# pxl-th/SLAM.jl

Hardware: AMD Instinct MI355X
Metric: frames/sec KITTI-05 stereo @1k kpts; local-BA ms/iter for 50-KF window (higher is better)
Workload: dtype f64

## Files before the change

slam.jl_amd/csrc/pyramid.hip:

```cpp
#include "common.hpp"
#include <cmath>
#include <cstdlib>
#include <mutex>
#include <tuple>
#include <utility>

#define LINE_THREADS 64

struct PlaneSet {
    double *p[4];
    const double *nrm[4];
    int coef[4];
    int fill0[4];
    const double *sq[4];
    int n;
    size_t zs;
};
#define PS_PICK(ps, f, pl) ((pl) == 0 ? (ps).f[0] : (pl) == 1 ? (ps).f[1] : (pl) == 2 ? (ps).f[2] : (ps).f[3])
__device__ __forceinline__ double *ps_plane(const PlaneSet &ps, int pl) { return PS_PICK(ps, p, pl) + (size_t)blockIdx.z * ps.zs; }
__device__ __forceinline__ const double *ps_nrm(const PlaneSet &ps, int pl) { return PS_PICK(ps, nrm, pl); }
__device__ __forceinline__ int ps_coef(const PlaneSet &ps, int pl) { return PS_PICK(ps, coef, pl); }
__device__ __forceinline__ bool ps_fill0(const PlaneSet &ps, int pl) { return PS_PICK(ps, fill0, pl) != 0; }
__device__ __forceinline__ const double *ps_sq(const PlaneSet &ps, int pl) { const double *q = PS_PICK(ps, sq, pl); return q ? q + (size_t)blockIdx.z * ps.zs : nullptr; }

// ... 236 lines not shown
    });
    const double uplus = iplus / k.inv1masum;
    const double vplus = uplus / k.inv1mbsum;
    const double d0 = w1 - uplus, d1 = w2 - uplus, d2 = w3 - uplus;
    const double vr0 = ((k.M[0] * d0 + k.M[1] * d1) + k.M[2] * d2) + vplus;
    const double vr1 = ((k.M[3] * d0 + k.M[4] * d1) + k.M[5] * d2) + vplus;
    const double vr2 = ((k.M[6] * d0 + k.M[7] * d1) + k.M[8] * d2) + vplus;
    double vA = vr0;
    double vB = ((w2 + a1 * vA) + a2 * vr1) + a3 * vr2;
    double vC = ((w3 + a1 * vB) + a2 * vA) + a3 * vr1;
    double v1 = vC, v2 = vB, v3 = vA;
    const double scale = k.scale;
    io.fence();
    if (nrm) {
        io.st(n - 1, (vA * scale) / nrm[(long)(n - 1) * nrm_s]);
        io.st(n - 2, (vB * scale) / nrm[(long)(n - 2) * nrm_s]);
        io.st(n - 3, (vC * scale) / nrm[(long)(n - 3) * nrm_s]);
        for (int i = n - 4; i >= 0; i--) {
            const double t = ((io.ld_dst(i) + a1 * v1) + a2 * v2) + a3 * v3;
            io.st(i, (t * scale) / nrm[(long)i * nrm_s]);
            v3 = v2; v2 = v1; v1 = t;
        }
        return;
    }
    io.st(n - 1, vA * scale); io.st(n - 2, vB * scale); io.st(n - 3, vC * scale);
    io.template sweep<-1>(n - 4, n - 3, true, [&](double x) {
        const double t = ((x + a1 * v1) + a2 * v2) + a3 * v3;
        v3 = v2; v2 = v1; v1 = t;
        return t * scale;
    });
}

template <int NB>
__global__ __launch_bounds__(LINE_THREADS) void k_iir_cols(PlaneSet ps, const double *src0, int H, int W, int P, IIRPair cf)
{
    if (src0) src0 += (size_t)blockIdx.z * ps.zs;
    __shared__ __attribute__((aligned(16))) double tile[64 * COL_LS];
    const int pl = blockIdx.y;
    ColIO<NB> io;
    io.dst = ps_plane(ps, pl); io.src = (pl == 0 && src0) ? src0 : io.dst;
    io.H = H; io.W = W; io.P = P; io.x0 = blockIdx.x * LINE_THREADS; io.lds = tile; io.slo = 0; io.shi = W - 1;
    iir_line(io, H, ps_coef(ps, pl) == 0 ? cf.c[0] : cf.c[1], ps_fill0(ps, pl), nullptr, 0);
}

__global__ __launch_bounds__(LINE_THREADS) void k_iir_rows(PlaneSet ps, int H, int W, int P, IIRPair cf)
{
    const int y = blockIdx.x * LINE_THREADS + threadIdx.x, pl = blockIdx.y;
    if (y >= H) return;
    RowIO io; io.src = ps_plane(ps, pl) + y; io.dst = ps_plane(ps, pl) + y; io.s = P;
    const double *nrm = ps_nrm(ps, pl);
    iir_line(io, W, ps_coef(ps, pl) == 0 ? cf.c[0] : cf.c[1], ps_fill0(ps, pl), nrm ? nrm + y : nullptr, P);
}

#define CK_B 32
struct RowResize { double *dst; int Hd, Wd, Pd; };
__device__ __forceinline__ double dpp_pair_next(double v)
{
    int lo = __double2loint(v), hi = __double2hiint(v);
    lo = __builtin_amdgcn_update_dpp(0, lo, 0xF5, 0xF, 0xF, true);
    hi = __builtin_amdgcn_update_dpp(0, hi, 0xF5, 0xF, 0xF, true);
    return __hiloint2double(hi, lo);
}
#define RCK_LD(ptr) __builtin_nontemporal_load(ptr)
#define RCK_ST(ptr, v) __builtin_nontemporal_store(v, ptr)
#define CK_LD(ptr) (*(ptr))
#define CK_ST(ptr, v) (*(ptr) = (v))
__global__ __launch_bounds__(LINE_THREADS) void k_iir_rows_ck(PlaneSet ps, int H, int W, int P, IIRPair cf, double *ck, RowResize rz)
{
    const int y = blockIdx.x * LINE_THREADS + threadIdx.x, pl = blockIdx.y;
    if (y >= H) return;
    const bool resize = pl == 0 && rz.dst != nullptr;
    const double rsx = (double)W / (double)(rz.Wd > 0 ? rz.Wd : 1), rox = 1 - 0.5 - rsx * (1 - 0.5);
    int xo = rz.Wd, c0 = -1; double fx = 0.0, tprev = 0.0;
    double *rzp = resize ? rz.dst + (size_t)blockIdx.z * ps.zs + (y >> 1) : nullptr;
    const bool exact2 = 2 * rz.Wd == W;
    auto rz_target = [&]() {
        if (xo < 1) { c0 = -1; return; }
        if (exact2) { c0 = 2 * xo - 2; fx = 0.5; return; }
        const double c = rsx * xo + rox;
        int ixx = (int)floor(c);
        if (ixx > W - 1) ixx = W - 1;
        if (ixx < 1) ixx = 1;
        fx = c - ixx;
        c0 = __builtin_amdgcn_readfirstlane(ixx - 1);
    };
    if (resize) rz_target();
    auto emit = [&](int x, double val) {
        if (x == c0) {
            const double h = (1 - fx) * val + fx * tprev;
            const double hn = dpp_pair_next(h);
            const double fy = 0.5;
            const double o = (1 - fy) * h + fy * hn;
            if ((y & 1) == 0) rzp[(size_t)(xo - 1) * rz.Pd] = o;
            xo--; rz_target();
        }
        tprev = val;
    };
    const size_t nlines = (size_t)gridDim.z * gridDim.y * gridDim.x * LINE_THREADS;
    const size_t lineid = ((size_t)blockIdx.z * gridDim.y + pl) * gridDim.x * LINE_THREADS + y;
    double *p = ps_plane(ps, pl) + y;
    const long s = P;
    const int n = W;
    const IIRCoef &k = ps_coef(ps, pl) == 0 ? cf.c[0] : cf.c[1];
    const bool fill0 = ps_fill0(ps, pl);
    const double a1 = k.a1, a2 = k.a2, a3 = k.a3, scale = k.scale;
    const double x0 = p[0];
    const double iminus = fill0 ? 0.0 : x0, iplus = fill0 ? 0.0 : p[(long)(n - 1) * s];
    const double uminus = iminus / k.inv1masum;
    const double o0 = ((x0 + a1 * uminus) + a2 * uminus) + a3 * uminus;
    const double o1 = ((p[s] + a1 * o0) + a2 * uminus) + a3 * uminus;
    const double o2 = ((p[2 * s] + a1 * o1) + a2 * o0) + a3 * uminus;
    const int m = n - 6, nb = (m + CK_B - 1) / CK_B;
    double w3 = o0, w2 = o1, w1 = o2;
    double cur[CK_B], nxt[CK_B];
    auto load_x = [&](int j, double *buf) {
        const double *q = p + (long)(3 + j * CK_B) * s;
        const int len = n - (3 + j * CK_B);
        if (len >= CK_B) {
#pragma unroll
            for (int e = 0; e < CK_B; e++) buf[e] = RCK_LD(q + (long)e * s);
        } else {
#pragma unroll
            for (int e = 0; e < CK_B; e++) buf[e] = e < len ? q[(long)e * s] : 0.0;
        }
    };
    const int nfull = (n - 3) / CK_B;
    const int rem = (n - 3) - nfull * CK_B;
    load_x(0, cur);
    for (int j = 0; j < nfull; j++) {
        load_x(j + 1, nxt);
        if (j > 0 && j < nb) { double *c = ck + ((size_t)j * 3) * nlines + lineid; CK_ST(c, w1); CK_ST(c + nlines, w2); CK_ST(c + 2 * nlines, w3); }
#pragma unroll
        for (int e = 0; e < CK_B; e++) { const double t = ((cur[e] + a1 * w1) + a2 * w2) + a3 * w3; w3 = w2; w2 = w1; w1 = t; }
#pragma unroll
        for (int e = 0; e < CK_B; e++) cur[e] = nxt[e];
    }
    {
        if (nfull > 0 && nfull < nb) { double *c = ck + ((size_t)nfull * 3) * nlines + lineid; CK_ST(c, w1); CK_ST(c + nlines, w2); CK_ST(c + 2 * nlines, w3); }
#pragma unroll
        for (int e = 0; e < CK_B; e++)
            if (e < rem) { const double t = ((cur[e] + a1 * w1) + a2 * w2) + a3 * w3; w3 = w2; w2 = w1; w1 = t; }
    }
    const bool have_last = nfull == nb - 1;
    const double uplus = iplus / k.inv1masum, vplus = uplus / k.inv1mbsum;
    const double d0 = w1 - uplus, d1 = w2 - uplus, d2 = w3 - uplus;
    const double vr0 = ((k.M[0] * d0 + k.M[1] * d1) + k.M[2] * d2) + vplus;
    const double vr1 = ((k.M[3] * d0 + k.M[4] * d1) + k.M[5] * d2) + vplus;
    const double vr2 = ((k.M[6] * d0 + k.M[7] * d1) + k.M[8] * d2) + vplus;
    const double vA = vr0;
    const double vB = ((w2 + a1 * vA) + a2 * vr1) + a3 * vr2;
    const double vC = ((w3 + a1 * vB) + a2 * vA) + a3 * vr1;
    double v1 = vC, v2 = vB, v3 = vA;
    __builtin_amdgcn_fence(__ATOMIC_RELEASE, "workgroup"); __builtin_amdgcn_fence(__ATOMIC_ACQUIRE, "workgroup");
    if (resize) { emit(n - 1, vA * scale); emit(n - 2, vB * scale); emit(n - 3, vC * scale); }
    else { p[(long)(n - 1) * s] = vA * scale; p[(long)(n - 2) * s] = vB * scale; p[(long)(n - 3) * s] = vC * scale; }
    double f1n = 0, f2n = 0, f3n = 0, f1 = 0, f2 = 0, f3 = 0;
    auto load_ck = [&](int j, double &g1, double &g2, double &g3) {
        if (j > 0) { const double *c = ck + ((size_t)j * 3) * nlines + lineid; g1 = CK_LD(c); g2 = CK_LD(c + nlines); g3 = CK_LD(c + 2 * nlines); }
        else { g1 = o2; g2 = o1; g3 = o0; }
    };
    if (nb > 0) {
        const int j = nb - 1, a = 3 + j * CK_B, len = m - j * CK_B;
        if (!have_last) load_x(j, cur);
        load_ck(j, f1, f2, f3);
        if (j > 0) { load_x(j - 1, nxt); load_ck(j - 1, f1n, f2n, f3n); }
#pragma unroll
        for (int e = 0; e < CK_B; e++)
            if (e < len) { const double t = ((cur[e] + a1 * f1) + a2 * f2) + a3 * f3; f3 = f2; f2 = f1; f1 = t; cur[e] = t; }
#pragma unroll
        for (int e = CK_B - 1; e >= 0; e--)
            if (e < len) { const double t = ((cur[e] + a1 * v1) + a2 * v2) + a3 * v3; v3 = v2; v2 = v1; v1 = t; cur[e] = t * scale; if (resize) emit(a + e, cur[e]); }
        double *q = p + (long)a * s;
        if (!resize) {
#pragma unroll
            for (int e = 0; e < CK_B; e++) if (e < len) RCK_ST(q + (long)e * s, cur[e]);
        }
#pragma unroll
        for (int e = 0; e < CK_B; e++) cur[e] = nxt[e];
        f1 = f1n; f2 = f2n; f3 = f3n;
    }
    for (int j = nb - 2; j >= 0; j--) {
        if (j > 0) { load_x(j - 1, nxt); load_ck(j - 1, f1n, f2n, f3n); }
#pragma unroll
        for (int e = 0; e < CK_B; e++) { const double t = ((cur[e] + a1 * f1) + a2 * f2) + a3 * f3; f3 = f2; f2 = f1; f1 = t; cur[e] = t; }
#pragma unroll
        for (int e = CK_B - 1; e >= 0; e--) { const double t = ((cur[e] + a1 * v1) + a2 * v2) + a3 * v3; v3 = v2; v2 = v1; v1 = t; cur[e] = t * scale; if (resize) emit(3 + j * CK_B + e, cur[e]); }
        double *q = p + (long)(3 + j * CK_B) * s;
        if (!resize) {
#pragma unroll
            for (int e = 0; e < CK_B; e++) RCK_ST(q + (long)e * s, cur[e]);
        }
#pragma unroll
        for (int e = 0; e < CK_B; e++) cur[e] = nxt[e];
        f1 = f1n; f2 = f2n; f3 = f3n;
    }
    {
        double t = ((o2 + a1 * v1) + a2 * v2) + a3 * v3; v3 = v2; v2 = v1; v1 = t; if (resize) emit(2, t * scale); else p[2 * s] = t * scale;
        t = ((o1 + a1 * v1) + a2 * v2) + a3 * v3; v3 = v2; v2 = v1; v1 = t; if (resize) emit(1, t * scale); else p[s] = t * scale;
        t = ((o0 + a1 * v1) + a2 * v2) + a3 * v3; if (resize) emit(0, t * scale); else p[0] = t * scale;
    }
}

__global__ __launch_bounds__(LINE_THREADS) void k_iir_cols_ck(PlaneSet ps, const double *src0, int H, int W, int P, IIRPair cf, double *ck)
{
    if (src0) src0 += (size_t)blockIdx.z * ps.zs;
    __shared__ __attribute__((aligned(16))) double tile[64 * COL_LS];
    const int pl = blockIdx.y, lane = threadIdx.x & 63;
    ColIO<2> io;
    const double *sqsrc = ps_sq(ps, pl);
    const bool sq = sqsrc != nullptr;
    io.dst = ps_plane(ps, pl); io.src = sq ? sqsrc : ((pl == 0 && src0) ? src0 : io.dst);
    io.H = H; io.W = W; io.P = P; io.x0 = blockIdx.x * LINE_THREADS; io.lds = tile; io.slo = 0; io.shi = W - 1; io.nt = true;
    const size_t nlines = (size_t)gridDim.z * gridDim.y * gridDim.x * LINE_THREADS;
    const size_t lineid = (((size_t)blockIdx.z * gridDim.y + pl) * gridDim.x + blockIdx.x) * LINE_THREADS + lane;
    const int n = H;
    const IIRCoef &k = ps_coef(ps, pl) == 0 ? cf.c[0] : cf.c[1];
    const bool fill0 = ps_fill0(ps, pl);
    const double a1 = k.a1, a2 = k.a2, a3 = k.a3, scale = k.scale;
    auto in = [&](double v) { return sq ? v * v : v; };
    const double x0 = in(io.ld_src(0));
    const double iminus = fill0 ? 0.0 : x0, iplus = fill0 ? 0.0 : in(io.ld_src(n - 1));
    const double uminus = iminus / k.inv1masum;
    const double o0 = ((x0 + a1 * uminus) + a2 * uminus) + a3 * uminus;
    const double o1 = ((in(io.ld_src(1)) + a1 * o0) + a2 * uminus) + a3 * uminus;
    const double o2 = ((in(io.ld_src(2)) + a1 * o1) + a2 * o0) + a3 * uminus;
    double w3 = o0, w2 = o1, w1 = o2;
    double raw[32], x[32];
    {
        const int NT = ((n - 1) >> 4) + 1;
        io.tile_load(io.src, 0, raw);
        for (int t = 0; t < NT; t++) {
            const int rb = t << 4;
            io.lds_put_tile(raw); io.template lds_get_col<+1>(x);
            if (sq) {
#pragma unroll
                for (int e = 0; e < 16; e++) x[e] = x[e] * x[e];
            }
            if (t + 1 < NT) io.tile_load(io.src, rb + 16, raw);
            if ((t & 1) == 0 && t >= 2) { double *c = ck + ((size_t)(t >> 1) * 3) * nlines + lineid; c[0] = w1; c[nlines] = w2; c[2 * nlines] = w3; }
            if (rb >= 3 && rb + 15 <= n - 1) {
#pragma unroll
                for (int e = 0; e < 16; e++) { const double tt = ((x[e] + a1 * w1) + a2 * w2) + a3 * w3; w3 = w2; w2 = w1; w1 = tt; }
            } else {
#pragma unroll
                for (int e = 0; e < 16; e++) { const int row = rb + e; if (row >= 3 && row <= n - 1) { const double tt = ((x[e] + a1 * w1) + a2 * w2) + a3 * w3; w3 = w2; w2 = w1; w1 = tt; } }
            }
        }
    }
    const double uplus = iplus / k.inv1masum, vplus = uplus / k.inv1mbsum;
    const double d0 = w1 - uplus, d1 = w2 - uplus, d2 = w3 - uplus;
    const double vr0 = ((k.M[0] * d0 + k.M[1] * d1) + k.M[2] * d2) + vplus;
    const double vr1 = ((k.M[3] * d0 + k.M[4] * d1) + k.M[5] * d2) + vplus;
    const double vr2 = ((k.M[6] * d0 + k.M[7] * d1) + k.M[8] * d2) + vplus;
// ... 9 lines not shown
        if (2 * b + 1 < ntile) io.tile_load(io.src, (b << 5) + 16, raw + 16);
    };
    if (n - 4 >= 3) load_block(NBk - 1);
    io.st(n - 1, vA * scale); io.st(n - 2, vB * scale); io.st(n - 3, vC * scale);
    for (int b = NBk - 1; b >= 0 && n - 4 >= 3; b--) {
        const int rb = b << 5, lo = rb > 3 ? rb : 3, hi = rb + 31 < n - 4 ? rb + 31 : n - 4;
        const bool two = 2 * b + 1 < ntile;
        io.lds_put_tile(raw); io.template lds_get_col<+1>(x);
        if (two) { io.lds_put_tile(raw + 16); io.template lds_get_col<+1>(x + 16); }
        if (sq) {
#pragma unroll
            for (int e = 0; e < 32; e++) x[e] = x[e] * x[e];
        }
        if (b > 0) load_block(b - 1);
        double f1, f2, f3;
        if (b > 0) { const double *c = ck + ((size_t)b * 3) * nlines + lineid; f1 = c[0]; f2 = c[nlines]; f3 = c[2 * nlines]; }
        else { f1 = o2; f2 = o1; f3 = o0; }
        if (lo == rb && hi == rb + 31) {
#pragma unroll
            for (int e = 0; e < 32; e++) { const double tt = ((x[e] + a1 * f1) + a2 * f2) + a3 * f3; f3 = f2; f2 = f1; f1 = tt; x[e] = tt; }
#pragma unroll
            for (int e = 31; e >= 0; e--) { const double tt = ((x[e] + a1 * v1) + a2 * v2) + a3 * v3; v3 = v2; v2 = v1; v1 = tt; x[e] = tt * scale; }
        } else {
#pragma unroll
            for (int e = 0; e < 32; e++) { const int row = rb + e; if (row >= lo && row <= hi) { const double tt = ((x[e] + a1 * f1) + a2 * f2) + a3 * f3; f3 = f2; f2 = f1; f1 = tt; x[e] = tt; } }
#pragma unroll
            for (int e = 31; e >= 0; e--) { const int row = rb + e; if (row >= lo && row <= hi) { const double tt = ((x[e] + a1 * v1) + a2 * v2) + a3 * v3; v3 = v2; v2 = v1; v1 = tt; x[e] = tt * scale; } }
        }
        double u[16];
        io.template lds_put_col<+1>(x); io.lds_get_tile(u);
        io.tile_store(rb, u, lo, hi, !(lo <= rb && hi >= rb + 15));
        if (two && hi >= rb + 16) {
            io.template lds_put_col<+1>(x + 16); io.lds_get_tile(u);
            io.tile_store(rb + 16, u, lo, hi, !(lo <= rb + 16 && hi >= rb + 31));
        }
    }
    {
        double tt = ((o2 + a1 * v1) + a2 * v2) + a3 * v3; v3 = v2; v2 = v1; v1 = tt; io.st(2, tt * scale);
        tt = ((o1 + a1 * v1) + a2 * v2) + a3 * v3; v3 = v2; v2 = v1; v1 = tt; io.st(1, tt * scale);
        tt = ((o0 + a1 * v1) + a2 * v2) + a3 * v3; io.st(0, tt * scale);
    }
}

#define CF4_COLS 62
struct ColsFusedArgs {
    const double *L;
    double *T;
    double *Iy, *Ix, *Qyy, *Qxx, *Qyx;
    int H, W, P; size_t zs;
    int src_kind; const void *const *srctab;
    double *tot; int tot_stride;
    int dec;
};

__device__ __forceinline__ double wave_prev(double v)
{
    int lo = __double2loint(v), hi = __double2hiint(v);
    lo = __builtin_amdgcn_update_dpp(lo, lo, 0x138, 0xF, 0xF, false);
    hi = __builtin_amdgcn_update_dpp(hi, hi, 0x138, 0xF, 0xF, false);
    return __hiloint2double(hi, lo);
}
__device__ __forceinline__ double wave_next(double v)
{
    int lo = __double2loint(v), hi = __double2hiint(v);
    lo = __builtin_amdgcn_update_dpp(lo, lo, 0x130, 0xF, 0xF, false);
    hi = __builtin_amdgcn_update_dpp(hi, hi, 0x130, 0xF, 0xF, false);
    return __hiloint2double(hi, lo);
}

template <bool TOL>
__device__ __forceinline__ double iir3(double x, double a1, double w1, double a2, double w2, double a3, double w3)
{
    if (TOL) return __builtin_fma(a1, w1, __builtin_fma(a2, w2, __builtin_fma(a3, w3, x)));
    return ((x + a1 * w1) + a2 * w2) + a3 * w3;
}
template <bool TOL>
__device__ __forceinline__ void scharr_pair(double a, double b, double c, double &d, double &s)
{
    const double dk[3] = {-1.0 / 2, 0.0 / 2, 1.0 / 2}, sk[3] = {3.0 / 16, 10.0 / 16, 3.0 / 16};
    if (TOL) { d = 0.5 * (c - a); s = __builtin_fma(sk[0], a + c, sk[1] * b); return; }
    double dd = 0.0; dd += a * dk[0]; dd += b * dk[1]; dd += c * dk[2];
    double ss = 0.0; ss += a * sk[0]; ss += b * sk[1]; ss += c * sk[2];
    d = dd; s = ss;
}
template <int ROLE, int N, bool TOL = false>
__device__ __forceinline__ void cf4_inputs(double *x, double top, double bot, int rb, int H, bool edgeL, bool edgeR, double *g)
{
    const double dk[3] = {-1.0 / 2, 0.0 / 2, 1.0 / 2}, sk[3] = {3.0 / 16, 10.0 / 16, 3.0 / 16};
    double a = top;
#pragma unroll
    for (int e = 0; e < N; e++) {
        const int row = rb + e;
        const double b = x[e];
        double c = e + 1 < N ? x[e + 1] : bot;
        const double aa = row == 0 ? b : a;
        c = row == H - 1 ? b : c;
        double iy = 0.0, ix = 0.0;
        double d, s;
        scharr_pair<TOL>(aa, b, c, d, s);
        if (ROLE == 1 || ROLE == 3) {
            double dl = wave_prev(d), dr = wave_next(d);
            dl = edgeL ? d : dl; dr = edgeR ? d : dr;
            if (TOL) iy = __builtin_fma(sk[0], dl + dr, sk[1] * d);
            else { iy += dl * sk[0]; iy += d * sk[1]; iy += dr * sk[2]; }
        }
        if (ROLE == 2 || ROLE == 3) {
            double sl = wave_prev(s), sr = wave_next(s);
            sl = edgeL ? s : sl; sr = edgeR ? s : sr;
            if (TOL) ix = 0.5 * (sr - sl);
            else { ix += sl * dk[0]; ix += s * dk[1]; ix += sr * dk[2]; }
        }
        double prod;
        if (ROLE == 1) { prod = iy * iy; g[e] = iy; }
        else if (ROLE == 2) { prod = ix * ix; g[e] = ix; }
        else prod = iy * ix;
        asm volatile("" : "+v"(prod));
        x[e] = prod;
        a = b;
    }
}

// ... 1154 lines not shown
    if (ixx > Ws - 1) ixx = Ws - 1;
    if (iy < 1) iy = 1;
    if (ixx < 1) ixx = 1;
    const double fy = r - iy, fx = c - ixx;
    const double *p = src + (size_t)(iy - 1) + (size_t)(ixx - 1) * Ps;
    const int dy = Hs > 1 ? 1 : 0; const size_t dx = Ws > 1 ? (size_t)Ps : 0;
    const double r0 = (1 - fx) * p[0] + fx * p[dx];
    const double r1 = (1 - fx) * p[dy] + fx * p[dy + dx];
    dst[(size_t)(y - 1) + (size_t)(x - 1) * Pd] = (1 - fy) * r0 + fy * r1;
}

__global__ __launch_bounds__(256) void k_u8_to_f64(double *dst, const unsigned char *src, int H, int W, int P)
{
    const size_t i = (size_t)blockIdx.x * 256 + threadIdx.x;
    if (i < (size_t)H * W) dst[i % H + (i / H) * P] = (double)src[i] / 255.0;
}

#define BATCH_MAX 128
struct ImgPtrs { const double *p[BATCH_MAX]; };
__global__ __launch_bounds__(256) void k_gather_images(ImgPtrs src, double *dst, int H, int W, int P, size_t zs)
{
    const size_t i = (size_t)blockIdx.x * 256 + threadIdx.x;
    if (i < (size_t)H * W) dst[(size_t)blockIdx.z * zs + i % H + (i / H) * P] = src.p[blockIdx.z][i];
}
struct ImgPtrsU8 { const unsigned char *p[BATCH_MAX]; };
__global__ __launch_bounds__(256) void k_gather_images_u8(ImgPtrsU8 src, double *dst, int H, int W, int P, size_t zs)
{
    const size_t i = (size_t)blockIdx.x * 256 + threadIdx.x;
    if (i < (size_t)H * W) dst[(size_t)blockIdx.z * zs + i % H + (i / H) * P] = (double)src.p[blockIdx.z][i] / 255.0;
}
__global__ __launch_bounds__(256) void k_unpitch(double *dst, const double *src, int H, int W, int P)
{
    const size_t i = (size_t)blockIdx.x * 256 + threadIdx.x;
    if (i < (size_t)H * W) dst[i] = src[i % H + (i / H) * P];
}

__global__ __launch_bounds__(256) void k_fill(double *p, size_t n, double v)
{
    const size_t i = (size_t)blockIdx.x * 256 + threadIdx.x;
    if (i < n) p[i] = v;
}

static inline int tol_batch_min_s()
{
    static const int v = [] { const char *e = getenv("SLAMHIP_TOL_BATCH_MIN_S"); return e ? atoi(e) : 4; }();
    return v;
}
static inline size_t ck_min_bytes()
{
    const char *e = getenv("SLAMHIP_CK_MIN_MB");
    return e ? (size_t)atol(e) << 20 : (size_t)40 << 20;
}
static inline dim3 lines_grid(int nlines, int nplanes, int S = 1) { return dim3((nlines + LINE_THREADS - 1) / LINE_THREADS, nplanes, S); }

static void make_view(slam_pyr *p)
{
    p->view.levels = p->levels;
    for (int l = 0; l < p->levels; l++) {
        LevelView &v = p->view.lv[l];
        v.L = p->plane(0, l); v.Iy = p->plane(1, l); v.Ix = p->plane(2, l);
        v.Iyy = p->plane(3, l); v.Ixx = p->plane(4, l); v.Iyx = p->plane(5, l);
        v.H = p->H[l]; v.W = p->W[l]; v.P = p->P[l];
    }
}

static int build_norm(slam_ctx *ctx, slam_pyr *p, double sigma)
{
    if (p->norm && p->norm_sigma == sigma) return SLAM_OK;
    if (!p->norm) HIP_TRY(ctx, hipMalloc((void **)&p->norm, ((size_t)p->off[p->levels] + (size_t)64 * p->P[0]) * 8));
    IIRPair cf; cf.c[0] = slam_iir_coef(sigma); cf.c[1] = cf.c[0];
    for (int l = 0; l + 1 < p->levels; l++) {
        double *N = p->norm + p->off[l];
        size_t n = (size_t)p->P[l] * p->W[l];
        hipLaunchKernelGGL(k_fill, dim3((n + 255) / 256), dim3(256), 0, ctx->stream, N, n, 1.0);
        PlaneSet ps = {}; ps.p[0] = N; ps.coef[0] = 0; ps.fill0[0] = 1; ps.n = 1;
        hipLaunchKernelGGL(k_iir_cols<3>, lines_grid(p->W[l], 1), dim3(LINE_THREADS), 0, ctx->stream, ps, (const double *)nullptr, p->H[l], p->W[l], p->P[l], cf);
        hipLaunchKernelGGL(k_iir_rows, lines_grid(p->H[l], 1), dim3(LINE_THREADS), 0, ctx->stream, ps, p->H[l], p->W[l], p->P[l], cf);
    }
    HIP_TRY(ctx, hipGetLastError());
    p->norm_sigma = sigma;
    return SLAM_OK;
}

static void mat3_pow(const IIRCoef &k, int e, double P[9])
{
    double M[9] = {k.a1, k.a2, k.a3, 1, 0, 0, 0, 1, 0}, R[9] = {1, 0, 0, 0, 1, 0, 0, 0, 1}, T[9];
    auto mul = [&](const double *A, const double *B, double *C) {
        for (int i = 0; i < 3; i++) for (int j = 0; j < 3; j++) { double t = 0; for (int m = 0; m < 3; m++) t += A[3 * i + m] * B[3 * m + j]; C[3 * i + j] = t; } };
    while (e > 0) {
        if (e & 1) { mul(R, M, T); memcpy(R, T, sizeof R); }
        mul(M, M, T); memcpy(M, T, sizeof M);
        e >>= 1;
    }
    memcpy(P, R, sizeof R);
}
static inline int seg_len(int n, int nseg_max) { int sl = (n + nseg_max - 1) / nseg_max; return sl < 4 ? 4 : sl; }
static void seg_pow(const IIRPair &cf, int n, int SL, SegPow &sp)
{
    const int nseg = (n + SL - 1) / SL, len_last = n - (nseg - 1) * SL;
    for (int c = 0; c < 2; c++) {
        for (int q = 1; q <= PAR_G; q++) mat3_pow(cf.c[c], SL * q, sp.P[c][q - 1]);
        mat3_pow(cf.c[c], len_last - 1, sp.Plast[c]);
    }
}

static int rt_seg_len(int n, int *ns)
{
    static const int menu[] = {4, 6, 8, 10, 12, 16, 20, 24, 32, 40};
    *ns = RT_NS;
    for (int m : menu) if ((n + m - 1) / m <= RT_NS && n >= 2 * m) return m;
    *ns = 2 * RT_NS;
    for (int m : {24, 32}) if ((n + m - 1) / m <= 2 * RT_NS && n >= 2 * m) return m;
    return 0;
}
static void rt_seg_pow(const IIRPair &cf, int SL, SegPow &sp)
{
    for (int c = 0; c < 2; c++) {
        for (int q = 1; q <= PAR_G; q++) mat3_pow(cf.c[c], SL * q, sp.P[c][q - 1]);
        mat3_pow(cf.c[c], SL - 1, sp.Plast[c]);
    }
}
enum { LN_MAIN = 0, LN_AUX = 1, LN_SIDE0 = 2, LN_COUNT = 2 + SLAM_MAX_LEVELS };
struct BuildSink {
    hipStream_t st = nullptr;
    hipGraph_t graph = nullptr;
    bool forked = false;
    hipGraphNode_t last[LN_COUNT] = {}, fork_dep[LN_COUNT] = {};
    hipError_t err = hipSuccess;
    template <typename Tup, size_t... I> static void addr_of(Tup &t, void **out, std::index_sequence<I...>) { ((out[I] = (void *)&std::get<I>(t)), ...); }
    template <typename... KA, typename... A>
    void launch(void (*kern)(KA...), dim3 grid, dim3 block, size_t lds, int lane, A &&...a)
    {
        if (!graph) { hipLaunchKernelGGL(kern, grid, block, lds, st, std::forward<A>(a)...); return; }
        std::tuple<KA...> args(std::forward<A>(a)...);
        void *ptrs[sizeof...(KA)];
        addr_of(args, ptrs, std::index_sequence_for<KA...>{});
        hipKernelNodeParams np = {};
        np.func = (void *)kern; np.gridDim = grid; np.blockDim = block; np.sharedMemBytes = (unsigned)lds; np.kernelParams = ptrs; np.extra = nullptr;
        const int ln = forked ? lane : LN_MAIN;
        hipGraphNode_t deps[2]; int nd = 0;
        if (last[ln]) deps[nd++] = last[ln];
        if (ln != LN_MAIN && fork_dep[ln] && fork_dep[ln] != last[ln]) deps[nd++] = fork_dep[ln];
        hipGraphNode_t node = nullptr;
        const hipError_t e = hipGraphAddKernelNode(&node, graph, nd ? deps : nullptr, (size_t)nd, &np);
        if (e != hipSuccess) { if (err == hipSuccess) err = e; return; }
        last[ln] = node;
        if (ln != LN_MAIN) fork_dep[ln] = nullptr;
    }
    void fork(int ln = LN_AUX) { if (graph && forked) fork_dep[ln] = last[LN_MAIN]; }
    bool lanes() const { return graph && forked; }
};

static void launch_level(slam_ctx *ctx, slam_pyr *p, int mode, const IIRPair &cf, BuildSink &B, bool spans, int S, int src_kind, bool target, int l, int z0, int Sall, bool fast)
{
    const size_t zs = p->zstride, zo = (size_t)z0 * zs;
    const int border_mode = (mode == 0) ? 1 : 0;
    {
        const int H = p->H[l], W = p->W[l], P = p->P[l];
        LevelView v = p->view.lv[l];
        v.L += zo; v.Iy += zo; v.Ix += zo; v.Iyy += zo; v.Ixx += zo; v.Iyx += zo;
        const bool has_next = l + 1 < p->levels;
        double *T = p->tmp + p->off[l] + zo;
        double *nextL = has_next ? p->view.lv[l + 1].L + zo : nullptr;
        if (target && l >= 1) {
            if (!has_next) return;
            PlaneSet pt = {}; pt.p[0] = T; pt.coef[0] = 0; pt.fill0[0] = (mode == 0); pt.nrm[0] = nullptr; pt.n = 1; pt.zs = zs;
            const bool ckr = (mode != 3 || Sall >= tol_batch_min_s()) && p->ck != nullptr && mode != 0 && W >= 64 && H >= 64 && (size_t)Sall * 4 * H * W * 8 >= ck_min_bytes();
            if (ckr) B.launch(k_iir_cols_ck, lines_grid(W, 1, S), dim3(LINE_THREADS), 0, LN_MAIN, pt, (const double *)v.L, H, W, P, cf, p->ck);
            else B.launch(k_iir_cols<2>, lines_grid(W, 1, S), dim3(LINE_THREADS), 0, LN_MAIN, pt, (const double *)v.L, H, W, P, cf);
            static const bool no_rr = getenv("SLAMHIP_NO_ROWS_RESIZE") != nullptr;
            const bool rr = ckr && (H & 1) == 0 && !no_rr;
            RowResize rzt = {};
            if (rr) { rzt.dst = nextL; rzt.Hd = p->H[l + 1]; rzt.Wd = p->W[l + 1]; rzt.Pd = p->P[l + 1]; }
            if (ckr) B.launch(k_iir_rows_ck, lines_grid(H, 1, S), dim3(LINE_THREADS), 0, LN_MAIN, pt, H, W, P, cf, p->ck, rzt);
            else B.launch(k_iir_rows, lines_grid(H, 1, S), dim3(LINE_THREADS), 0, LN_MAIN, pt, H, W, P, cf);
            if (!rr)
                B.launch(k_resize, dim3(((size_t)p->H[l + 1] * p->W[l + 1] + 255) / 256, 1, S), dim3(256), 0, LN_MAIN,
                                   nextL, p->H[l + 1], p->W[l + 1], p->P[l + 1], (const double *)T, H, W, P, zs);
            return;
        }
        const int np_ = has_next ? 4 : 3;
        static const bool no_ck_cols = getenv("SLAMHIP_NO_CK_COLS") != nullptr;
        const bool ck_cols = !fast && p->ck != nullptr && mode != 0 && H >= 64 && (size_t)Sall * np_ * H * W * 8 >= ck_min_bytes() && !no_ck_cols;
        static const bool no_sq = getenv("SLAMHIP_NO_SQ_FUSE") != nullptr;
        const bool fuse_sq = ck_cols && !no_sq;
        static const bool no_cols_fused = getenv("SLAMHIP_NO_COLS_FUSED") != nullptr;
        const bool cols_fused = fuse_sq && !no_cols_fused;
        static const bool no_topo = getenv("SLAMHIP_TOPOLOGY") == nullptr;
        const bool topo = S == 1 && Sall == 1 && has_next && !cols_fused && B.lanes() && !no_topo;
        const int side = topo ? LN_SIDE0 + l : LN_MAIN;
        const int side_cum = topo ? LN_SIDE0 + l : LN_AUX;
        if (topo) B.fork(side);
        auto emit_scharr = [&](int lane_) {
            static const int sch1 = [] { const char *e = getenv("SLAMHIP_SCHARR_XC1"); return e ? atoi(e) : 2; }();
            if (!cols_fused && S == 1 && sch1 == 4) B.launch(k_scharr_products<4>, dim3((H + 63) / 64, (W + 3) / 4, S), dim3(64), 0, lane_, v, border_mode, zs, fuse_sq ? 0 : 1);
            else if (!cols_fused && S == 1 && sch1 == 2) B.launch(k_scharr_products<2>, dim3((H + 63) / 64, (W + 1) / 2, S), dim3(64), 0, lane_, v, border_mode, zs, fuse_sq ? 0 : 1);
            else if (!cols_fused && S == 1 && sch1 == 1) B.launch(k_scharr_products<1>, dim3((H + 63) / 64, W, S), dim3(64), 0, lane_, v, border_mode, zs, fuse_sq ? 0 : 1);
            else if (!cols_fused && S == 1 && sch1 == 8) B.launch(k_scharr_products<8>, dim3((H + 63) / 64, (W + 7) / 8, S), dim3(64), 0, lane_, v, border_mode, zs, fuse_sq ? 0 : 1);
            else if (!cols_fused) B.launch(k_scharr_products<SCH_XC>, dim3((H + 63) / 64, (W + SCH_XC - 1) / SCH_XC, S), dim3(64), 0, lane_, v, border_mode, zs, fuse_sq ? 0 : 1);
        };
        emit_scharr(side);
        PlaneSet ps = {};
        int np = 0;
        if (has_next) { ps.p[np] = T; ps.coef[np] = 0; ps.fill0[np] = (mode == 0); ps.nrm[np] = (mode == 0) ? p->norm + p->off[l] : nullptr; np++; }
        ps.p[np] = v.Iyy; ps.coef[np] = 1; ps.sq[np] = fuse_sq ? v.Iy : nullptr; np++;
        ps.p[np] = v.Ixx; ps.coef[np] = 1; ps.sq[np] = fuse_sq ? v.Ix : nullptr; np++;
        ps.p[np] = v.Iyx; ps.coef[np] = 1; np++;
        ps.n = np; ps.zs = zs;
        const double *src0 = has_next ? (const double *)v.L : (const double *)nullptr;
        PlaneSet psT = {}, psQ = {};
        if (topo) {
            psT.p[0] = ps.p[0]; psT.coef[0] = ps.coef[0]; psT.fill0[0] = ps.fill0[0]; psT.nrm[0] = ps.nrm[0]; psT.n = 1; psT.zs = zs;
            for (int q = 0; q < 3; q++) { psQ.p[q] = ps.p[q + 1]; psQ.coef[q] = ps.coef[q + 1]; psQ.fill0[q] = ps.fill0[q + 1]; psQ.nrm[q] = ps.nrm[q + 1]; psQ.sq[q] = ps.sq[q + 1]; }
            psQ.n = 3; psQ.zs = zs;
        }
        PlaneSet pc = {};
        pc.p[0] = v.Iyy; pc.p[1] = v.Ixx; pc.p[2] = v.Iyx; pc.n = 3; pc.zs = zs;
        if (fast) {
            const int slc = seg_len(H, PAR_T / 8), slr = seg_len(W, PAR_T / 8);
            SegPow spc, spr;
            seg_pow(cf, H, slc, spc); seg_pow(cf, W, slr, spr);
            const dim3 gc((W + 7) / 8, np, S), gr((H + 7) / 8, np, S), gc3((W + 7) / 8, 3, S), gr3((H + 7) / 8, 3, S);
            static const bool seg_wide = getenv("SLAMHIP_SEG_WIDE") != nullptr;
            const int slc32 = seg_len(H, 32);
            const bool c32 = slc32 <= PAR_SLMAX && !seg_wide;
            SegPow spc32;
            if (c32) seg_pow(cf, H, slc32, spc32);
// ... 66 lines not shown
            ca.H = H; ca.W = W; ca.P = P; ca.zs = zs;
            ca.src_kind = l == 0 ? src_kind : 0; ca.srctab = (const void *const *)p->alloc->srctab + z0;
            size_t toff = 0;
            for (int q = 0; q < l; q++) toff += (size_t)3 * Sall * p->W[q];
            toff += (size_t)3 * z0 * W;
            ca.tot = tolb ? p->alloc->tot + toff : nullptr; ca.tot_stride = W;
            static const bool no_dec = getenv("SLAMHIP_NO_TOL_DEC") != nullptr;
            ca.dec = (tolb && has_next && (H & 1) == 0 && (P & 31) == 0 && !no_dec) ? 1 : 0;
            if (tolb && ca.dec) B.launch(k_cols_fused<true, true>, dim3((W + CF4_COLS - 1) / CF4_COLS, 1, S), dim3(256), 0, LN_MAIN, ca, cf, p->ck);
            else if (tolb) B.launch(k_cols_fused<true, false>, dim3((W + CF4_COLS - 1) / CF4_COLS, 1, S), dim3(256), 0, LN_MAIN, ca, cf, p->ck);
            else B.launch(k_cols_fused<false, false>, dim3((W + CF4_COLS - 1) / CF4_COLS, 1, S), dim3(256), 0, LN_MAIN, ca, cf, p->ck);
            if (tolb) {
                RowsTolArgs ra = {};
                int nr = 0;
                if (has_next) { ra.p[nr] = T; ra.coef[nr] = 0; ra.kind[nr] = 0; nr++; }
                ra.nq0 = nr;
                ra.p[nr] = v.Iyy; ra.coef[nr] = 1; ra.kind[nr] = 1; nr++;
                ra.p[nr] = v.Ixx; ra.coef[nr] = 1; ra.kind[nr] = 1; nr++;
                ra.p[nr] = v.Iyx; ra.coef[nr] = 1; ra.kind[nr] = 1; nr++;
                ra.n = nr; ra.zs = zs; ra.tot = ca.tot; ra.tot_stride = W;
                const bool rzf = has_next && (H & 1) == 0;
                ra.dec = ca.dec;
                if (rzf) { ra.rz.dst = nextL; ra.rz.Hd = p->H[l + 1]; ra.rz.Wd = p->W[l + 1]; ra.rz.Pd = p->P[l + 1]; }
                SegPow spr; rt_seg_pow(cf, slr_t, spr);
                static const int rt_dbg = getenv("SLAMHIP_RT_DBG") ? atoi(getenv("SLAMHIP_RT_DBG")) : 0; ra.dbg = rt_dbg;
                const dim3 gr((H + RT_R - 1) / RT_R, nr, S), bd(RT_R * rt_ns);
                auto go = [&]() {
                    if (rt_ns != RT_NS) {
                        if (slr_t == 24) B.launch((k_rows_tol<24, 2 * RT_NS, RT_R>), gr, bd, 0, LN_MAIN, ra, H, W, P, cf, spr);
                        else B.launch((k_rows_tol<32, 2 * RT_NS, RT_R>), gr, bd, 0, LN_MAIN, ra, H, W, P, cf, spr);
                        return;
                    }
#define RT_GO(SLV) B.launch((k_rows_tol<SLV, RT_NS, RT_R>), gr, bd, 0, LN_MAIN, ra, H, W, P, cf, spr)
                    switch (slr_t) { case 4: RT_GO(4); break; case 6: RT_GO(6); break; case 8: RT_GO(8); break; case 10: RT_GO(10); break; case 12: RT_GO(12); break;
                                     case 16: RT_GO(16); break; case 20: RT_GO(20); break; case 24: RT_GO(24); break; case 32: RT_GO(32); break; default: RT_GO(40); break; }
#undef RT_GO
                };
                if (spans) { ProfScope span(ctx, "k_iir_rows"); go(); } else go();
                if (has_next && !rzf)
                    B.launch(k_resize, dim3(((size_t)p->H[l + 1] * p->W[l + 1] + 255) / 256, 1, S), dim3(256), 0, LN_MAIN,
                                       nextL, p->H[l + 1], p->W[l + 1], p->P[l + 1], (const double *)T, H, W, P, zs);
                return;
            }
        }
        else if (ck_cols) B.launch(k_iir_cols_ck, lines_grid(W, np, S), dim3(LINE_THREADS), 0, LN_MAIN, ps, src0, H, W, P, cf, p->ck);
        else if (topo) {
            B.launch(k_iir_cols<3>, lines_grid(W, 1, S), dim3(LINE_THREADS), 0, LN_MAIN, psT, src0, H, W, P, cf);
            B.launch(k_iir_cols<3>, lines_grid(W, 3, S), dim3(LINE_THREADS), 0, side, psQ, (const double *)nullptr, H, W, P, cf);
        }
        else if (S == 1) B.launch(k_iir_cols<3>, lines_grid(W, np, S), dim3(LINE_THREADS), 0, LN_MAIN, ps, src0, H, W, P, cf);
        else B.launch(k_iir_cols<2>, lines_grid(W, np, S), dim3(LINE_THREADS), 0, LN_MAIN, ps, src0, H, W, P, cf);
        const bool ck_rows = p->ck != nullptr && mode != 0 && W >= 64 && (size_t)Sall * np * H * W * 8 >= ck_min_bytes();
        static const bool no_rows_resize = getenv("SLAMHIP_NO_ROWS_RESIZE") != nullptr;
        const bool rows_resize = ck_rows && has_next && (H & 1) == 0 && !no_rows_resize;
        RowResize rz = {};
        if (rows_resize) { rz.dst = nextL; rz.Hd = p->H[l + 1]; rz.Wd = p->W[l + 1]; rz.Pd = p->P[l + 1]; }
        static const bool no_rows_cum = getenv("SLAMHIP_NO_ROWS_CUM") != nullptr;
        static const bool no_fused_cum = getenv("SLAMHIP_NO_FUSED_CUM") != nullptr;
        const int cf_bands = (H + 63) / 64;
        if (!topo && Sall >= 8 && mode != 0 && W >= 64 && cf_bands <= CF_MAXW && p->alloc->rck != nullptr && !no_rows_cum && !no_fused_cum) {
            B.fork();
            if (has_next) {
                PlaneSet pT = {}; pT.p[0] = ps.p[0]; pT.coef[0] = ps.coef[0]; pT.fill0[0] = ps.fill0[0]; pT.n = 1; pT.zs = zs;
                if (spans) { ProfScope span(ctx, "k_iir_rows");
                    if (ck_rows) B.launch(k_iir_rows_ck, lines_grid(H, 1, S), dim3(LINE_THREADS), 0, LN_MAIN, pT, H, W, P, cf, p->ck, rz);
                    else B.launch(k_iir_rows, lines_grid(H, 1, S), dim3(LINE_THREADS), 0, LN_MAIN, pT, H, W, P, cf); }
                else if (ck_rows) B.launch(k_iir_rows_ck, lines_grid(H, 1, S), dim3(LINE_THREADS), 0, LN_MAIN, pT, H, W, P, cf, p->ck, rz);
                else B.launch(k_iir_rows, lines_grid(H, 1, S), dim3(LINE_THREADS), 0, LN_MAIN, pT, H, W, P, cf);
                if (!rows_resize)
                    B.launch(k_resize, dim3(((size_t)p->H[l + 1] * p->W[l + 1] + 255) / 256, 1, S), dim3(256), 0, LN_MAIN,
                                       nextL, p->H[l + 1], p->W[l + 1], p->P[l + 1], (const double *)T, H, W, P, zs);
            }
            PlaneSet pq = {};
            for (int q = 0; q < 3; q++) { pq.p[q] = ps.p[np - 3 + q]; pq.coef[q] = ps.coef[np - 3 + q]; pq.fill0[q] = ps.fill0[np - 3 + q]; }
            pq.n = 3; pq.zs = zs;
            const size_t lds = (size_t)cf_bands * RC_LDS_DOUBLES * sizeof(double);
            B.launch(k_rows_cum, dim3(1, 3, S), dim3(cf_bands * 64), lds, LN_AUX, pq, H, W, P, cf, p->alloc->rck);
            return;
        }
        if (topo) {
            B.launch(k_iir_rows, lines_grid(H, 1, S), dim3(LINE_THREADS), 0, LN_MAIN, psT, H, W, P, cf);
            B.launch(k_iir_rows, lines_grid(H, 3, S), dim3(LINE_THREADS), 0, side, psQ, H, W, P, cf);
        }
        else if (spans) { ProfScope span(ctx, "k_iir_rows");
            if (ck_rows) B.launch(k_iir_rows_ck, lines_grid(H, np, S), dim3(LINE_THREADS), 0, LN_MAIN, ps, H, W, P, cf, p->ck, rz);
            else B.launch(k_iir_rows, lines_grid(H, np, S), dim3(LINE_THREADS), 0, LN_MAIN, ps, H, W, P, cf); }
        else if (ck_rows) B.launch(k_iir_rows_ck, lines_grid(H, np, S), dim3(LINE_THREADS), 0, LN_MAIN, ps, H, W, P, cf, p->ck, rz);
        else B.launch(k_iir_rows, lines_grid(H, np, S), dim3(LINE_THREADS), 0, LN_MAIN, ps, H, W, P, cf);
        if (!topo) B.fork();
        if (has_next && !rows_resize)
            B.launch(k_resize, dim3(((size_t)p->H[l + 1] * p->W[l + 1] + 255) / 256, 1, S), dim3(256), 0, LN_MAIN,
                               nextL, p->H[l + 1], p->W[l + 1], p->P[l + 1], (const double *)T, H, W, P, zs);
        const int cf_seg = cf_bands <= CF_MAXW ? 1 : (cf_bands + CF_SEGW - 1) / CF_SEGW;
        if (Sall >= 8 && !no_fused_cum && (cf_seg == 1 || (p->alloc->xc != nullptr && cf_seg <= p->alloc->xseg))) {
            const int nw = cf_seg == 1 ? cf_bands : CF_SEGW;
            const size_t lds = ((size_t)nw * CF_W * CF_LS + (size_t)nw * 2 * CF_W) * sizeof(double);
            const size_t xo = (size_t)z0 * 3 * (size_t)(cf_seg > 1 ? cf_seg - 1 : 1);
            if (cf_seg == 1) B.launch(k_cum_fused<false>, dim3(1, 3, S), dim3(nw * 64), lds, LN_AUX, pc, H, W, P, (double *)nullptr, (int *)nullptr);
            else B.launch(k_cum_fused<true>, dim3(cf_seg, 3, S), dim3(nw * 64), lds, LN_AUX, pc, H, W, P, p->alloc->xc + xo * W, p->alloc->xf + xo);
            return;
        }
        if (S == 1) B.launch(k_cum_cols<3>, lines_grid(W, 3, S), dim3(LINE_THREADS), 0, side_cum, pc, H, W, P);
        else B.launch(k_cum_cols<2>, lines_grid(W, 3, S), dim3(LINE_THREADS), 0, LN_AUX, pc, H, W, P);
        B.launch(k_cum_rows, lines_grid(H, 3, S), dim3(LINE_THREADS), 0, S == 1 ? side_cum : LN_AUX, pc, H, W, P);
    }
}


static void launch_build(slam_ctx *ctx, slam_pyr *p, int mode, const IIRPair &cf, BuildSink &B, bool spans, int S = 1, int src_kind = 0, bool target = false)
{
    bool fast = mode == 3;
    if (fast && (seg_len(p->H[0], PAR_T / 8) > PAR_SLMAX || seg_len(p->W[0], PAR_T / 8) > PAR_SLMAX)) fast = false;
    if (fast && S >= tol_batch_min_s()) fast = false;
    static const int chunk_mb = [] { const char *v = getenv("SLAMHIP_PYR_CHUNK_MB"); return v ? atoi(v) : 0; }();
    for (int l = 0; l < p->levels; l++) {
        int C = S;
        if (chunk_mb > 0 && S >= 8 && mode != 0) {
            const size_t per_image = (size_t)4 * p->P[l] * p->W[l] * 8;
            const size_t want = (size_t)chunk_mb << 20;
            if (per_image * S > 2 * want) { C = (int)std::max<size_t>(4, want / per_image); C = std::min(C, S); }
        }
        for (int z0 = 0; z0 < S; z0 += C) launch_level(ctx, p, mode, cf, B, spans, std::min(C, S - z0), src_kind, target, l, z0, S, fast);
    }
}

static bool level0_fused(const slam_pyr *p, int mode, int S)
{
    static const bool off = getenv("SLAMHIP_NO_COLS_FUSED") != nullptr || getenv("SLAMHIP_NO_SQ_FUSE") != nullptr || getenv("SLAMHIP_NO_CK_COLS") != nullptr ||
                            getenv("SLAMHIP_NO_FUSED_INGEST") != nullptr;
    if (off || mode == 0 || p->ck == nullptr || p->alloc->srctab == nullptr || p->H[0] < 64) return false;
    if (mode == 3 && S < tol_batch_min_s() && !(seg_len(p->H[0], PAR_T / 8) > PAR_SLMAX || seg_len(p->W[0], PAR_T / 8) > PAR_SLMAX)) return false;
    const int np_ = p->levels > 1 ? 4 : 3;
    return (size_t)S * np_ * p->H[0] * p->W[0] * 8 >= ck_min_bytes();
}
__global__ void k_set_ptrs(const void **tab, ImgPtrs src)
{
    if (threadIdx.x < BATCH_MAX) tab[threadIdx.x] = src.p[threadIdx.x];
}

static int enqueue_build(slam_ctx *ctx, slam_pyr *p, int mode_flags, double sigma, int S = 1, int src_kind = 0)
// ... 284 lines not shown
```

Before: 23520.

## Fuse downsample resize into row IIR pass for odd-height pyramid levels

Adds an ODD template variant of the checkpointed row IIR kernel that also writes the bilinearly resized next pyramid level when the level height is odd. Previously that case fell back to a separate k_resize launch. The variant uses overlapping 63-row bands so wave_next can fetch the neighbouring row, and it computes horizontal taps per 32-element chunk. This removes one kernel and a full-plane reread for odd-height levels, in exchange for more complex index logic, one redundant lane per band, and a risk of subtle resize mismatches.

```diff
diff --git a/slam.jl_amd/csrc/pyramid.hip b/slam.jl_amd/csrc/pyramid.hip
--- a/slam.jl_amd/csrc/pyramid.hip
+++ b/slam.jl_amd/csrc/pyramid.hip
@@ -312,8 +312,24 @@
     iir_line(io, W, ps_coef(ps, pl) == 0 ? cf.c[0] : cf.c[1], ps_fill0(ps, pl), nrm ? nrm + y : nullptr, P);
 }
 
+__device__ __forceinline__ double wave_prev(double v)
+{
+    int lo = __double2loint(v), hi = __double2hiint(v);
+    lo = __builtin_amdgcn_update_dpp(lo, lo, 0x138, 0xF, 0xF, false);
+    hi = __builtin_amdgcn_update_dpp(hi, hi, 0x138, 0xF, 0xF, false);
+    return __hiloint2double(hi, lo);
+}
+__device__ __forceinline__ double wave_next(double v)
+{
+    int lo = __double2loint(v), hi = __double2hiint(v);
+    lo = __builtin_amdgcn_update_dpp(lo, lo, 0x130, 0xF, 0xF, false);
+    hi = __builtin_amdgcn_update_dpp(hi, hi, 0x130, 0xF, 0xF, false);
+    return __hiloint2double(hi, lo);
+}
+
 #define CK_B 32
 struct RowResize { double *dst; int Hd, Wd, Pd; };
+#define RZ_ODD_ROWS (LINE_THREADS - 1)
 __device__ __forceinline__ double dpp_pair_next(double v)
 {
     int lo = __double2loint(v), hi = __double2hiint(v);
@@ -325,14 +341,28 @@
 #define RCK_ST(ptr, v) __builtin_nontemporal_store(v, ptr)
 #define CK_LD(ptr) (*(ptr))
 #define CK_ST(ptr, v) (*(ptr) = (v))
-__global__ __launch_bounds__(LINE_THREADS) void k_iir_rows_ck(PlaneSet ps, int H, int W, int P, IIRPair cf, double *ck, RowResize rz)
-{
-    const int y = blockIdx.x * LINE_THREADS + threadIdx.x, pl = blockIdx.y;
+template <bool ODD>
+__device__ __forceinline__ void iir_rows_ck(const PlaneSet &ps, int H, int W, int P, const IIRPair &cf, double *ck, const RowResize &rz)
+{
+    const int pl = blockIdx.y;
+    const bool resize = ODD || (pl == 0 && rz.dst != nullptr);
+    const int slot = blockIdx.x * LINE_THREADS + threadIdx.x;
+    const int y = ODD ? blockIdx.x * RZ_ODD_ROWS + threadIdx.x : slot;
     if (y >= H) return;
-    const bool resize = pl == 0 && rz.dst != nullptr;
     const double rsx = (double)W / (double)(rz.Wd > 0 ? rz.Wd : 1), rox = 1 - 0.5 - rsx * (1 - 0.5);
     int xo = rz.Wd, c0 = -1; double fx = 0.0, tprev = 0.0;
-    double *rzp = resize ? rz.dst + (size_t)blockIdx.z * ps.zs + (y >> 1) : nullptr;
+    int yo = y >> 1; double fy = 0.5; bool rz_store = (y & 1) == 0;
+    if (ODD) {
+        yo = (y + 1) >> 1;
+        const double rsy = (double)H / (double)rz.Hd, roy = 1 - 0.5 - rsy * (1 - 0.5);
+        const double r = rsy * (yo + 1) + roy;
+        int iy = (int)floor(r);
+        if (iy > H - 1) iy = H - 1;
+        if (iy < 1) iy = 1;
+        fy = r - iy;
+        rz_store = yo < rz.Hd && iy - 1 == y && threadIdx.x < RZ_ODD_ROWS;
+    }
+    double *rzp = resize ? rz.dst + (size_t)blockIdx.z * ps.zs + yo : nullptr;
     const bool exact2 = 2 * rz.Wd == W;
     auto rz_target = [&]() {
         if (xo < 1) { c0 = -1; return; }
@@ -348,16 +378,22 @@
     auto emit = [&](int x, double val) {
         if (x == c0) {
             const double h = (1 - fx) * val + fx * tprev;
-            const double hn = dpp_pair_next(h);
-            const double fy = 0.5;
-            const double o = (1 - fy) * h + fy * hn;
-            if ((y & 1) == 0) rzp[(size_t)(xo - 1) * rz.Pd] = o;
+            if (ODD) {
+                const double hn = wave_next(h);
+                const double o = (1 - fy) * h + fy * hn;
+                if (rz_store) rzp[(size_t)(xo - 1) * rz.Pd] = o;
+            } else {
+                const double hn = dpp_pair_next(h);
+                const double fy2 = 0.5;
+                const double o = (1 - fy2) * h + fy2 * hn;
+                if ((y & 1) == 0) rzp[(size_t)(xo - 1) * rz.Pd] = o;
+            }
             xo--; rz_target();
         }
         tprev = val;
     };
     const size_t nlines = (size_t)gridDim.z * gridDim.y * gridDim.x * LINE_THREADS;
-    const size_t lineid = ((size_t)blockIdx.z * gridDim.y + pl) * gridDim.x * LINE_THREADS + y;
+    const size_t lineid = ((size_t)blockIdx.z * gridDim.y + pl) * gridDim.x * LINE_THREADS + slot;
     double *p = ps_plane(ps, pl) + y;
     const long s = P;
     const int n = W;
@@ -444,7 +480,28 @@
 #pragma unroll
         for (int e = 0; e < CK_B; e++) { const double t = ((cur[e] + a1 * f1) + a2 * f2) + a3 * f3; f3 = f2; f2 = f1; f1 = t; cur[e] = t; }
 #pragma unroll
-        for (int e = CK_B - 1; e >= 0; e--) { const double t = ((cur[e] + a1 * v1) + a2 * v2) + a3 * v3; v3 = v2; v2 = v1; v1 = t; cur[e] = t * scale; if (resize) emit(3 + j * CK_B + e, cur[e]); }
+        for (int e = CK_B - 1; e >= 0; e--) { const double t = ((cur[e] + a1 * v1) + a2 * v2) + a3 * v3; v3 = v2; v2 = v1; v1 = t; cur[e] = t * scale; if (!ODD && resize) emit(3 + j * CK_B + e, cur[e]); }
+        if (ODD) {
+            const int kb = (3 + j * CK_B + 1) >> 1;
+#pragma unroll
+            for (int mm = 0; mm < CK_B / 2; mm++) {
+                const int k1 = kb + mm + 1;
+                const double c = rsx * k1 + rox;
+                int ixx = (int)floor(c);
+                if (ixx > W - 1) ixx = W - 1;
+                if (ixx < 1) ixx = 1;
+                const double fxm = c - ixx;
+                const bool low = ixx == 2 * k1 - 2;
+                const double lft = low ? cur[2 * mm] : cur[2 * mm + 1];
+                const double rgt = low ? cur[2 * mm + 1] : (2 * mm + 2 < CK_B ? cur[2 * mm + 2 < CK_B ? 2 * mm + 2 : 0] : tprev);
+                const double h = (1 - fxm) * lft + fxm * rgt;
+                const double hn = wave_next(h);
+                const double o = (1 - fy) * h + fy * hn;
+                if (rz_store) rzp[(size_t)(k1 - 1) * rz.Pd] = o;
+            }
+            tprev = cur[0];
+            if (j == 0) { xo = kb; rz_target(); }
+        }
         double *q = p + (long)(3 + j * CK_B) * s;
         if (!resize) {
 #pragma unroll
@@ -459,6 +516,14 @@
         t = ((o1 + a1 * v1) + a2 * v2) + a3 * v3; v3 = v2; v2 = v1; v1 = t; if (resize) emit(1, t * scale); else p[s] = t * scale;
         t = ((o0 + a1 * v1) + a2 * v2) + a3 * v3; if (resize) emit(0, t * scale); else p[0] = t * scale;
     }
+}
+__global__ __launch_bounds__(LINE_THREADS) void k_iir_rows_ck(PlaneSet ps, int H, int W, int P, IIRPair cf, double *ck, RowResize rz)
+{
+    iir_rows_ck<false>(ps, H, W, P, cf, ck, rz);
+}
+__global__ __launch_bounds__(LINE_THREADS) void k_iir_rows_ck_odd(PlaneSet ps, int H, int W, int P, IIRPair cf, double *ck, RowResize rz)
+{
+    iir_rows_ck<true>(ps, H, W, P, cf, ck, rz);
 }
 
 __global__ __launch_bounds__(LINE_THREADS) void k_iir_cols_ck(PlaneSet ps, const double *src0, int H, int W, int P, IIRPair cf, double *ck)
@@ -574,21 +639,6 @@
     double *tot; int tot_stride;
     int dec;
 };
-
-__device__ __forceinline__ double wave_prev(double v)
-{
-    int lo = __double2loint(v), hi = __double2hiint(v);
-    lo = __builtin_amdgcn_update_dpp(lo, lo, 0x138, 0xF, 0xF, false);
-    hi = __builtin_amdgcn_update_dpp(hi, hi, 0x138, 0xF, 0xF, false);
-    return __hiloint2double(hi, lo);
-}
-__device__ __forceinline__ double wave_next(double v)
-{
-    int lo = __double2loint(v), hi = __double2hiint(v);
-    lo = __builtin_amdgcn_update_dpp(lo, lo, 0x130, 0xF, 0xF, false);
-    hi = __builtin_amdgcn_update_dpp(hi, hi, 0x130, 0xF, 0xF, false);
-    return __hiloint2double(hi, lo);
-}
 
 template <bool TOL>
 __device__ __forceinline__ double iir3(double x, double a1, double w1, double a2, double w2, double a3, double w3)
@@ -1849,6 +1899,14 @@
     return e ? (size_t)atol(e) << 20 : (size_t)40 << 20;
 }
 static inline dim3 lines_grid(int nlines, int nplanes, int S = 1) { return dim3((nlines + LINE_THREADS - 1) / LINE_THREADS, nplanes, S); }
+static inline int rz_odd_bands(int H) { return (H - 1 + RZ_ODD_ROWS - 1) / RZ_ODD_ROWS; }
+static inline bool rz_odd_ok(const slam_pyr *p, int l)
+{
+    static const bool off = getenv("SLAMHIP_NO_ROWS_RESIZE_ODD") != nullptr;
+    if (off || l + 1 >= p->levels) return false;
+    const int H = p->H[l], W = p->W[l], Wd = p->W[l + 1];
+    return H >= 3 && 2 * p->H[l + 1] - 1 == H && (W == 2 * Wd || W == 2 * Wd - 1) && rz_odd_bands(H) <= 4 * ((p->H[0] + LINE_THREADS - 1) / LINE_THREADS);
+}
 
 static void make_view(slam_pyr *p)
 {
@@ -1948,6 +2006,12 @@
     bool lanes() const { return graph && forked; }
 };
 
+static void launch_rows_ck(BuildSink &B, const PlaneSet &ps, int nplanes, int S, int H, int W, int P, const IIRPair &cf, double *ck, const RowResize &rz, bool odd)
+{
+    if (odd) B.launch(k_iir_rows_ck_odd, dim3(rz_odd_bands(H), 1, S), dim3(LINE_THREADS), 0, LN_MAIN, ps, H, W, P, cf, ck, rz);
+    else B.launch(k_iir_rows_ck, lines_grid(H, nplanes, S), dim3(LINE_THREADS), 0, LN_MAIN, ps, H, W, P, cf, ck, rz);
+}
+
 static void launch_level(slam_ctx *ctx, slam_pyr *p, int mode, const IIRPair &cf, BuildSink &B, bool spans, int S, int src_kind, bool target, int l, int z0, int Sall, bool fast)
 {
     const size_t zs = p->zstride, zo = (size_t)z0 * zs;
@@ -1966,10 +2030,11 @@
             if (ckr) B.launch(k_iir_cols_ck, lines_grid(W, 1, S), dim3(LINE_THREADS), 0, LN_MAIN, pt, (const double *)v.L, H, W, P, cf, p->ck);
             else B.launch(k_iir_cols<2>, lines_grid(W, 1, S), dim3(LINE_THREADS), 0, LN_MAIN, pt, (const double *)v.L, H, W, P, cf);
             static const bool no_rr = getenv("SLAMHIP_NO_ROWS_RESIZE") != nullptr;
-            const bool rr = ckr && (H & 1) == 0 && !no_rr;
+            const bool rr_odd = ckr && (H & 1) != 0 && !no_rr && rz_odd_ok(p, l);
+            const bool rr = (ckr && (H & 1) == 0 && !no_rr) || rr_odd;
             RowResize rzt = {};
             if (rr) { rzt.dst = nextL; rzt.Hd = p->H[l + 1]; rzt.Wd = p->W[l + 1]; rzt.Pd = p->P[l + 1]; }
-            if (ckr) B.launch(k_iir_rows_ck, lines_grid(H, 1, S), dim3(LINE_THREADS), 0, LN_MAIN, pt, H, W, P, cf, p->ck, rzt);
+            if (ckr) launch_rows_ck(B, pt, 1, S, H, W, P, cf, p->ck, rzt, rr_odd);
             else B.launch(k_iir_rows, lines_grid(H, 1, S), dim3(LINE_THREADS), 0, LN_MAIN, pt, H, W, P, cf);
             if (!rr)
                 B.launch(k_resize, dim3(((size_t)p->H[l + 1] * p->W[l + 1] + 255) / 256, 1, S), dim3(256), 0, LN_MAIN,
@@ -2142,9 +2207,14 @@
         else B.launch(k_iir_cols<2>, lines_grid(W, np, S), dim3(LINE_THREADS), 0, LN_MAIN, ps, src0, H, W, P, cf);
         const bool ck_rows = p->ck != nullptr && mode != 0 && W >= 64 && (size_t)Sall * np * H * W * 8 >= ck_min_bytes();
         static const bool no_rows_resize = getenv("SLAMHIP_NO_ROWS_RESIZE") != nullptr;
-        const bool rows_resize = ck_rows && has_next && (H & 1) == 0 && !no_rows_resize;
+        const bool rz_odd_cand = ck_rows && has_next && (H & 1) != 0 && !no_rows_resize;
+        bool rows_resize = ck_rows && has_next && (H & 1) == 0 && !no_rows_resize;
+        bool rows_odd = false;
         RowResize rz = {};
-        if (rows_resize) { rz.dst = nextL; rz.Hd = p->H[l + 1]; rz.Wd = p->W[l + 1]; rz.Pd = p->P[l + 1]; }
+        auto rz_decide = [&](int nplanes) {
+            if (rz_odd_cand && nplanes == 1 && rz_odd_ok(p, l)) rows_resize = rows_odd = true;
+            if (rows_resize) { rz.dst = nextL; rz.Hd = p->H[l + 1]; rz.Wd = p->W[l + 1]; rz.Pd = p->P[l + 1]; }
+        };
         static const bool no_rows_cum = getenv("SLAMHIP_NO_ROWS_CUM") != nullptr;
         static const bool no_fused_cum = getenv("SLAMHIP_NO_FUSED_CUM") != nullptr;
         const int cf_bands = (H + 63) / 64;
@@ -2152,10 +2222,11 @@
             B.fork();
             if (has_next) {
                 PlaneSet pT = {}; pT.p[0] = ps.p[0]; pT.coef[0] = ps.coef[0]; pT.fill0[0] = ps.fill0[0]; pT.n = 1; pT.zs = zs;
+                rz_decide(1);
                 if (spans) { ProfScope span(ctx, "k_iir_rows");
-                    if (ck_rows) B.launch(k_iir_rows_ck, lines_grid(H, 1, S), dim3(LINE_THREADS), 0, LN_MAIN, pT, H, W, P, cf, p->ck, rz);
+                    if (ck_rows) launch_rows_ck(B, pT, 1, S, H, W, P, cf, p->ck, rz, rows_odd);
                     else B.launch(k_iir_rows, lines_grid(H, 1, S), dim3(LINE_THREADS), 0, LN_MAIN, pT, H, W, P, cf); }
-                else if (ck_rows) B.launch(k_iir_rows_ck, lines_grid(H, 1, S), dim3(LINE_THREADS), 0, LN_MAIN, pT, H, W, P, cf, p->ck, rz);
+                else if (ck_rows) launch_rows_ck(B, pT, 1, S, H, W, P, cf, p->ck, rz, rows_odd);
                 else B.launch(k_iir_rows, lines_grid(H, 1, S), dim3(LINE_THREADS), 0, LN_MAIN, pT, H, W, P, cf);
                 if (!rows_resize)
                     B.launch(k_resize, dim3(((size_t)p->H[l + 1] * p->W[l + 1] + 255) / 256, 1, S), dim3(256), 0, LN_MAIN,
@@ -2168,14 +2239,15 @@
             B.launch(k_rows_cum, dim3(1, 3, S), dim3(cf_bands * 64), lds, LN_AUX, pq, H, W, P, cf, p->alloc->rck);
             return;
         }
+        if (!topo) rz_decide(np);
         if (topo) {
             B.launch(k_iir_rows, lines_grid(H, 1, S), dim3(LINE_THREADS), 0, LN_MAIN, psT, H, W, P, cf);
             B.launch(k_iir_rows, lines_grid(H, 3, S), dim3(LINE_THREADS), 0, side, psQ, H, W, P, cf);
         }
         else if (spans) { ProfScope span(ctx, "k_iir_rows");
-            if (ck_rows) B.launch(k_iir_rows_ck, lines_grid(H, np, S), dim3(LINE_THREADS), 0, LN_MAIN, ps, H, W, P, cf, p->ck, rz);
+            if (ck_rows) launch_rows_ck(B, ps, np, S, H, W, P, cf, p->ck, rz, rows_odd);
             else B.launch(k_iir_rows, lines_grid(H, np, S), dim3(LINE_THREADS), 0, LN_MAIN, ps, H, W, P, cf); }
-        else if (ck_rows) B.launch(k_iir_rows_ck, lines_grid(H, np, S), dim3(LINE_THREADS), 0, LN_MAIN, ps, H, W, P, cf, p->ck, rz);
+        else if (ck_rows) launch_rows_ck(B, ps, np, S, H, W, P, cf, p->ck, rz, rows_odd);
         else B.launch(k_iir_rows, lines_grid(H, np, S), dim3(LINE_THREADS), 0, LN_MAIN, ps, H, W, P, cf);
         if (!topo) B.fork();
         if (has_next && !rows_resize)
```

New measurement: 23830, median of 6. +1.3%, better.
